# NikoBiele/RayTraceHeatTransfer.jl

Measured on AMD Instinct MI355X. Metric: Mrays/sec (exchange-factor trace), 101×101 grey κ=1 enclosure, 1/2/4/8 GPUs, higher is better.
Workload: dtype f64; 1 GPU; 101x101 grey kappa=1 sigma_s=0 unit-square enclosure (BASELINE configs[1]); 1e+08 rays per GPU, emitter rows sharded over 1 GPU(s); n_emitters=10605, rays_per_emitter=9429, parallelism=emitter-rows x1 (one process per GPU), devices_visible=1, seed=1

## Files before the change

raytraceheattransfer.jl_amd/csrc/rthx_api.cpp:

```cpp
#define RTHX_HOST_ONLY_TU 1
#include <hip/hip_runtime.h>

#include <algorithm>
#include <array>
#include <chrono>
#include <cmath>
#include <cstdio>
#include <cstdlib>
#include <cstring>
#include <map>
#include <mutex>
#include <string>
#include <thread>
#include <vector>

#include "../../include/rthx.h"
#include "rthx_grid.h"
#include "rthx_kernels.h"

#include "rthx_common.h"
#include "rthx_domain.h"

using rthx::DevBuf;
using rthx::HostBuf;
// ... 144 lines not shown
extern "C" __attribute__((visibility("default"))) int rthx_debug_neg_log(const double* u, int64_t n, double* out) {
  if ((!u || !out) && n > 0) return -1;
  std::vector<double> t(rthx::kTableDoubles);
  rthx::fill_tables(t.data());
  for (int64_t k = 0; k < n; ++k) out[k] = rthx::neg_log_tab(u[k], t.data() + rthx::kLogTableOffset);
  return 0;
}

extern "C" __attribute__((visibility("default"))) int rthx_debug_neg_log_u32(const uint32_t* w, int64_t n,
                                                                             double* out) {
  if ((!w || !out) && n > 0) return -1;
  std::vector<double> t(rthx::kTableDoubles);
  rthx::fill_tables(t.data());
  for (int64_t k = 0; k < n; ++k) out[k] = rthx::neg_log_u32(w[k], t.data() + rthx::kLogTableOffset);
  return 0;
}

extern "C" __attribute__((visibility("default"))) int rthx_debug_wall_candidate(double s, double d, int32_t form) {
  const double as = std::fabs(s), ad = std::fabs(d);
  switch (form) {
    case 0: return rthx::wall_candidate(s, d) ? 1 : 0;
    case 1: return (ad >= 1e-10 && as * ad > 0.0) ? 1 : 0;
    case 2: return (as / ad > 0.0 && ad >= 1e-10) ? 1 : 0;
    default: return -1;
  }
}

extern "C" __attribute__((visibility("default"))) int rthx_debug_sin_theta_sweep(int32_t device, uint32_t w_begin,
                                                                                 uint64_t n, uint64_t* n_diff,
                                                                                 uint64_t* first_diff) {
  if (!n_diff || !first_diff) return fail(RTHX_EINVAL, "null output");
  if ((uint64_t)w_begin + n > (1ull << 32)) return fail(RTHX_EINVAL, "word range past 2^32");
  hipStream_t stream = nullptr;
  RTHX_TRY(rthx::open_device(device, &stream));
  DevBuf buf;
  HIP_TRY(buf.reserve(2 * sizeof(unsigned long long)), "hipMalloc (sin theta sweep)");
  unsigned long long h[2] = {0ull, ~0ull};
  HIP_TRY(hipMemcpyAsync(buf.p, h, sizeof(h), hipMemcpyHostToDevice, stream), "hipMemcpy (sin theta sweep)");
  HIP_TRY(rthx::launch_sin_theta_sweep(w_begin, n, (unsigned long long*)buf.p, stream), "sin_theta_sweep_kernel");
  HIP_TRY(hipMemcpyAsync(h, buf.p, sizeof(h), hipMemcpyDeviceToHost, stream), "hipMemcpy (sin theta sweep)");
  HIP_TRY(hipStreamSynchronize(stream), "hipStreamSynchronize (sin theta sweep)");
  *n_diff = h[0];
  *first_diff = h[1];
  return RTHX_OK;
}

// ... 435 lines not shown
      const int w2 = (w + 1) % dom->c_nv[c];
      const std::pair<double, double> a{v[2 * w], v[2 * w + 1]}, b{v[2 * w2], v[2 * w2 + 1]};
      return a < b ? Key{a.first, a.second, b.first, b.second} : Key{b.first, b.second, a.first, a.second};
    };
    std::map<Key, std::vector<std::pair<size_t, int>>> walls;
    for (size_t c = 0; c < nc; ++c)
      for (int w = 0; w < dom->c_nv[c]; ++w) walls[key_of(c, w)].push_back({c, w});
    const std::vector<uint32_t> flagged = mask;
    for (size_t c = 0; c < nc; ++c)
      for (int w = 0; w < dom->c_nv[c]; ++w)
        if ((flagged[c] >> w) & 1u)
          for (const auto& o : walls[key_of(c, w)])
            if (!((dom->c_solid[o.first] >> o.second) & 1u)) mask[o.first] |= 1u << o.second;
  }
  rthx::DeviceGuard keep_device;
  HIP_TRY(hipSetDevice(dom->device), "hipSetDevice");
  HIP_TRY(hipMemcpyAsync(dom->d_mirror, mask.data(), nc * sizeof(uint32_t), hipMemcpyHostToDevice, dom->stream),
          "hipMemcpy mirror masks");
  HIP_TRY(hipStreamSynchronize(dom->stream), "mirror masks");
  dom->n_mirror = n;
  return RTHX_OK;
}

RTHX_EXPORT int rthx_domain_get_mirror_walls(const rthx_domain* dom, int64_t* n_mirror) {
  if (!dom || !n_mirror) return fail(RTHX_EINVAL, "null domain or output");
  *n_mirror = dom->n_mirror;
  return RTHX_OK;
}

RTHX_EXPORT void rthx_domain_destroy(rthx_domain* dom) {
  if (!dom) return;
  (void)hipSetDevice(dom->device);
  (void)hipStreamSynchronize(dom->stream);
  delete dom;
}

RTHX_EXPORT int rthx_result_create(rthx_result** out) {
  if (!out) return fail(RTHX_EINVAL, "null out");
  *out = new (std::nothrow) rthx_result();
  return *out ? RTHX_OK : fail(RTHX_ENOMEM, "host allocation failed");
}

RTHX_EXPORT void rthx_result_destroy(rthx_result* res) { delete res; }

namespace rthx {

// ... 111 lines not shown
             p.cl_offset + (size_t)dom->D.cl.bytes + rthx::kStaticLdsBytes <= rthx::kMaxLdsBytes && !no_clds) {
    p.clds = 1;
    p.lds_bytes = p.cl_offset + (size_t)dom->D.cl.bytes;
  }
  if (single && dom->D.lat.bytes > 0 && !p.recording &&
      p.cl_offset + (size_t)dom->D.lat.bytes + rthx::kStaticLdsBytes <= rthx::kMaxLdsBytes) {
    p.clds = 1;
    p.lds_bytes = p.cl_offset + (size_t)dom->D.lat.bytes;
  }
  if (p.n_rows * p.split >= (1ll << 31)) return fail(RTHX_ERANGE, "too many workgroups in one call");
  p.uniform = dom->uniform_beta[a->bin] > -0.1;
  return RTHX_OK;
}

rthx::LaunchCfg launch_of(const rthx_domain* dom, const rthx_trace_args* a, const TracePlan& p) {
  rthx::LaunchCfg L{};
  L.D = dom->d_dom;
  L.lds_bytes = p.lds_bytes;
  L.uniform = p.uniform;
  L.tally = p.tally;
  L.threads = (int)env_int("RTHX_TRACE_THREADS", 0, 0, rthx::kMaxTraceThreads);
  L.faithful = (a->flags & RTHX_FLAG_FAITHFUL_SAMPLING) != 0;
  L.mirror = p.mirror;
  L.single = dom->single_convex && !p.mirror;
  L.clds = p.clds;
  L.axis = dom->axis_rect && !p.mirror && !env_flag("RTHX_NO_AXIS");
  L.T.split = (int32_t)p.split;
  L.T.n_rows = p.n_rows;
  L.rec.n = p.recording ? 1 : 0;
  return L;
}

int plan_trace_split(const rthx_domain* dom, const rthx_trace_args* a, TracePlan& p) {
  int rc = plan_trace(dom, a, p);
  if (rc || p.split > 1 || p.recording || p.n_rows == 0 || p.R < 2 * kSplitMinRays) return rc;
  int64_t slots = 0;
  rthx::LaunchCfg L = launch_of(dom, a, p);
  L.slots = &slots;
  HIP_TRY(rthx::launch_trace(L), "trace kernel occupancy query");
  if (slots <= 0) return RTHX_OK;
  return plan_trace(dom, a, p, slots);
}

int run_trace(rthx_domain* dom, const rthx_trace_args* a, const TracePlan& p, rthx_result* res, bool lookback,
              const rthx::RecordParams& rec, int64_t totals[rthx::kLbTotals], float* ms_trace, float* ms_pack,
              bool async = false, bool check_prev = false) {
// ... 730 lines not shown
```

raytraceheattransfer.jl_amd/csrc/rthx_device.h:

```cpp
#pragma once

#include <hip/hip_runtime.h>
#include <stdint.h>

#if defined(__HIP_DEVICE_COMPILE__) && !defined(RTHX_HOST_ONLY_TU)
#define RTHX_GLOBAL __attribute__((address_space(1)))
#else
#define RTHX_GLOBAL
#endif
#define RTHX_LDS __attribute__((address_space(3)))

namespace rthx {

struct DevGrid {
  double ox, oy;
  double inv_x, inv_y;
  int32_t nx, ny;
  int32_t cell_base;
  int32_t reserved;
};

struct alignas(16) DevPoly {
  double x[4], y[4];
  double nx[4], ny[4];
// ... 199 lines not shown
constexpr uint64_t kLogOff = 0x3FE6000000000000ull;

__host__ __device__ __forceinline__ double neg_log_tab(double u, const double* tab) {
  const uint64_t ix = dbits(u);
  const uint64_t tmp = ix - kLogOff;
  const int i = (int)((tmp >> 45) & (kLogTable - 1));
  const int32_t k = (int32_t)(uint32_t)(tmp >> 32) >> 20;
  const double z = bitsd(ix - (tmp & 0xFFF0000000000000ull));
  const double invc = tab[4 * i], t_hi = tab[4 * i + 1], t_lo = tab[4 * i + 2];
  const double r = __builtin_fma(z, invc, -1.0);
  double q = __builtin_fma(r, 1.0 / 7.0, -1.0 / 6.0);
  q = __builtin_fma(r, q, sconst(1.0 / 5.0));
  q = __builtin_fma(r, q, -1.0 / 4.0);
  q = __builtin_fma(r, q, sconst(1.0 / 3.0));
  q = __builtin_fma(r, q, -0.5);
  const double l1p = __builtin_fma(r * r, q, r);
  const double kd = (double)k;
  const double hi = __builtin_fma(-kd, 6.93147180369123816490e-01, t_hi);
  const double lo = __builtin_fma(-kd, 1.90821492927058770002e-10, t_lo) - l1p;
  const double v = hi + lo;
  return u > 0.0 ? v : __builtin_inf();
}

__host__ __device__ __forceinline__ double neg_log_u32(uint32_t w, const double* tab) {
  static_assert((uint32_t)kLogOff == 0u, "the high-word form needs a zero low word");
  const uint64_t ix = dbits((double)w);
  const uint32_t ix_hi = (uint32_t)(ix >> 32);
  const uint32_t tmp_hi = ix_hi - (uint32_t)(kLogOff >> 32);
  const uint32_t i32 = ((tmp_hi >> 13) & (uint32_t)(kLogTable - 1)) << 5;
  const int32_t k = ((int32_t)tmp_hi >> 20) - 32;
  const double z = bitsd(((uint64_t)(ix_hi - (tmp_hi & 0xFFF00000u)) << 32) | (uint32_t)ix);
  const double* const te = (const double*)((const char*)tab + i32);
  const double invc = te[0], t_hi = te[1], t_lo = te[2];
  const double r = __builtin_fma(z, invc, -1.0);
  double q = fma_cc(r, 1.0 / 7.0, -1.0 / 6.0);
  q = __builtin_fma(r, q, sconst(1.0 / 5.0));
  q = __builtin_fma(r, q, -1.0 / 4.0);
  q = __builtin_fma(r, q, sconst(1.0 / 3.0));
  q = __builtin_fma(r, q, -0.5);
  const double l1p = __builtin_fma(r * r, q, r);
  const double kd = (double)k;
  const double hi = __builtin_fma(-kd, 6.93147180369123816490e-01, t_hi);
  const double lo = __builtin_fma(-kd, 1.90821492927058770002e-10, t_lo) - l1p;
  const double v = hi + lo;
  return w != 0u ? v : __builtin_inf();
}

__device__ __forceinline__ double div_pos(double n, double d) {
  double r = __builtin_amdgcn_rcp(d);
  double e = __builtin_fma(-d, r, 1.0);
  r = __builtin_fma(r, e, r);
  e = __builtin_fma(-d, r, 1.0);
  r = __builtin_fma(r, e, r);
  const double q = n * r;
  const double rem = __builtin_fma(-d, q, n);
  return __builtin_fma(rem, r, q);
}

__device__ __forceinline__ double sqrt_unit(double x) {
  const double y = __builtin_amdgcn_rsq(__builtin_fmax(x, 0x1.0p-1000));
  double g = x * y, h = 0.5 * y;
  const double r = __builtin_fma(-h, g, 0.5);
  g = __builtin_fma(g, r, g);
  h = __builtin_fma(h, r, h);
  double d = __builtin_fma(-g, g, x);
  g = __builtin_fma(d, h, g);
  d = __builtin_fma(-g, g, x);
// ... 554 lines not shown
  bool gas;
  bool lost;
  bool cold;
};

__device__ __forceinline__ int lattice_walk(const double RTHX_LDS* b, int nm1, int i, double x) {
#pragma unroll 1
  while (true) {
    const bool dn = i > 0 && x < b[i];
    const bool up = !dn && i < nm1 && !(x < b[i + 1]);
    if (!(dn | up)) break;
    i += dn ? -1 : 1;
  }
  return (b[i] <= x && x < b[i + 1]) ? i : -1;
}

__device__ __forceinline__ int lattice_guess(double x, double x0, double inv, int nm1) {
  int i;
  __asm__("v_cvt_i32_f64 %0, %1" : "=v"(i) : "v"(__dmul_rn(x - x0, inv)));
  __asm__("v_med3_i32 %0, %1, 0, %2" : "=v"(i) : "v"(i), "v"(nm1));
  return i;
}

template <bool INSIDE>
__device__ __forceinline__ int lat_ray_fast(const DevDomain& D, double eta, const SingleCoarse& sc,
                                            const char RTHX_LDS* lat_base, bool identity, bool cold0, LatRay& r) {
  const double ox = r.px, oy = r.py, dx = r.dx, dy = r.dy, S = r.S;
  const double cx0 = sc.poly.x[0], cx1 = sc.poly.x[1], cy0 = sc.poly.y[0], cy1 = sc.poly.y[2];
  const bool xdn = dx < 0.0, ydn = dy < 0.0;
  const bool y_first = ydn | xdn;
  double u;
  int k;
  if (INSIDE) {
    const double xb = xdn ? cx0 : cx1, yb = ydn ? cy0 : cy1;
    const double sx = xb - ox, sy = yb - oy;
    const bool vx = wall_candidate(sx, dx), vy = wall_candidate(sy, dy);
    const double cx = __dmul_rn(fabs(sx), fabs(dy)), cy = __dmul_rn(fabs(sy), fabs(dx));
    const bool xw = vx & (!vy | (y_first & (cx < cy)) | (!y_first & !(cy < cx)));
    const bool any = vx | vy;
    const double q = div_pos(fabs(xw ? sx : sy), fabs(xw ? dx : dy));
    u = any ? q : __builtin_inf();
    k = any ? (xw ? (xdn ? 3 : 1) : (ydn ? 0 : 2)) : 0;
  } else {
    if (cx0 <= ox && ox < cx1 && cy0 <= oy && oy < cy1)
      u = dist_in_box(ox, oy, dx, dy, xdn ? cx0 : cx1, ydn ? cy0 : cy1, k);
    else
      u = dist_to_box(ox, oy, dx, dy, cx0, cx1, cy0, cy1, k);
  }
  const bool gas = S < u;
  const bool wall = !gas & (((sc.solid >> k) & 1u) != 0u);
  const bool lost = !(gas | wall);
  const double t = (gas ? S : u) - eta;
  const double px = ox + __dmul_rn(t, dx);
  const double py = oy + __dmul_rn(t, dy);
  r.px = px;
  r.py = py;
  r.gas = gas;
  r.lost = lost;
  const LatGrid& G = sc.lat;
  const double RTHX_LDS* xs = (const double RTHX_LDS*)lat_base;
  const double RTHX_LDS* ys = (const double RTHX_LDS*)(lat_base + G.off_ys);
  const int i = lattice_guess(px, G.x0, G.inv_x, G.nxm1);
  const int j = lattice_guess(py, G.y0, G.inv_y, G.nym1);
  const double xlo = xs[i], xhi = xs[i + 1], ylo = ys[j], yhi = ys[j + 1];
  const bool hit = (xlo <= px) & (px < xhi) & (ylo <= py) & (py < yhi);
  int f = lat_cell(i, j, G.nx);
  if (!identity) f = D.lat_map[f];
  const double sx = (xdn ? xlo : xhi) - px, sy = (ydn ? ylo : yhi) - py;
  const bool vx = wall_candidate(sx, dx), vy = wall_candidate(sy, dy);
  const double cx = __dmul_rn(fabs(sx), fabs(dy)), cy = __dmul_rn(fabs(sy), fabs(dx));
  const bool xw = vx & (!vy | (y_first & (cx < cy)) | (!y_first & !(cy < cx)));
  const int wl = xw ? (xdn ? 3 : 1) : (ydn ? 0 : 2);
  int surf = -1;
  if (wall) surf = ld_off32(D.f_surf, ((uint32_t)f << 4) + ((uint32_t)wl << 2));
  const int a = gas ? sc.n_surfaces + f : surf;
  r.cold = cold0 | lost | !hit | (wall & !(vx | vy)) | (a < 0);
  return a;
}

__device__ __forceinline__ int lat_ray_fixup(const DevDomain& D, const SingleCoarse& sc,
                                             const char RTHX_LDS* lat_base, bool identity, const LatRay& r) {
  if (r.lost) return -1;
  const double px = r.px, py = r.py, dx = r.dx, dy = r.dy;
  const LatGrid& G = sc.lat;
  const double RTHX_LDS* xs = (const double RTHX_LDS*)lat_base;
  const double RTHX_LDS* ys = (const double RTHX_LDS*)(lat_base + G.off_ys);
  const int i = lattice_walk(xs, G.nxm1, lattice_guess(px, G.x0, G.inv_x, G.nxm1), px);
  const int j = lattice_walk(ys, G.nym1, lattice_guess(py, G.y0, G.inv_y, G.nym1), py);
  if (i < 0 || j < 0) return -1;
  int f = lat_cell(i, j, G.nx);
  if (!identity) f = D.lat_map[f];
  if (r.gas) return sc.n_surfaces + f;
  const int w = box_hit_in(px, py, dx, dy, dx < 0.0 ? xs[i] : xs[i + 1], dy < 0.0 ? ys[j] : ys[j + 1]).wall;
  return ld_off32(D.f_surf, ((uint32_t)f << 4) + ((uint32_t)w << 2));
}

template <class T>
__device__ __forceinline__ T ld(const T RTHX_LDS* p) { return *(const T*)p; }
template <class T>
__device__ __forceinline__ T ld(const T RTHX_GLOBAL* p) { return *p; }
// ... 400 lines not shown
  px = px + __dmul_rn(t, r.dx);
  py = py + __dmul_rn(t, r.dy);
}

__device__ __forceinline__ int end_ml(const DevDomain& D, const MLatLds& L, const MLatLayout& G, const MBox& B,
                                      double px, double py, double dx, double dy, bool gas) {
  const MCoarse m = ld(L.cinfo + L.cmap[B.b]);
  int i, j;
  const int fg = ml_fine(L, G, m, px, py, i, j);
  if (fg < 0) return -1;
  if (gas) return D.n_surfaces + fg;
  const int w = box_hit_in(px, py, dx, dy, dx < 0.0 ? L.xs[i] : L.xs[i + 1], dy < 0.0 ? L.ys[j] : L.ys[j + 1]).wall;
  return D.f_surf[4 * fg + w];
}

template <bool UNIFORM, bool FAITHFUL>
__device__ __forceinline__ double free_path(const TraceParams& P, const double* tabs, double u) {
  if (UNIFORM)
    return FAITHFUL ? (P.beta_uniform > 0 ? -log(u) / P.beta_uniform : __builtin_inf())
                    : neg_log_tab(u, tabs + kLogTableOffset) * tabs[kTabInvBeta];
  return FAITHFUL ? -log(u) : neg_log_tab(u, tabs + kLogTableOffset);
}

template <bool UNIFORM, bool FAITHFUL, bool LATRAY = false>
__device__ __forceinline__ double free_path_u32(const TraceParams& P, const double* tabs, uint32_t w,
                                                const SingleCoarse* sc = nullptr) {
  if (FAITHFUL) return free_path<UNIFORM, true>(P, tabs, u32(w));
  const double l = neg_log_u32(w, tabs + kLogTableOffset);
  if (UNIFORM) return l * (LATRAY ? sc->inv_beta : tabs[kTabInvBeta]);
  return l;
}

template <int EK = kEmitAny>
__device__ __forceinline__ bool emitter_surface(const Emitter& e) { return EK == kEmitAny ? e.surface : false; }

template <int EK = kEmitAny>
__device__ __forceinline__ RayWords ray_words(const TraceParams& P, const Emitter& e, uint32_t g, uint32_t r,
                                              bool have_pw, uint32_t pw, bool faithful) {
  RayWords rw;
  philox_words(r, g, 0u, (uint32_t)P.bin, P.key0, P.key1, rw.a);
  rw.pw = 0u;
  rw.sw = 0u;
  if (!emitter_surface<EK>(e)) {
    if (have_pw) {
      rw.pw = pw;
    } else {
      uint32_t b[4];
      philox_words(r >> 2, g, 1u, (uint32_t)P.bin, P.key0, P.key1, b);
      const uint32_t j = r & 3u;
      rw.pw = j == 0 ? b[0] : j == 1 ? b[1] : j == 2 ? b[2] : b[3];
    }
    if (EK == kEmitVolRect ? faithful : (e.need_sel || (faithful && e.nv == 4))) {
      uint32_t c[4];
      philox_words(r, g, 2u, (uint32_t)P.bin, P.key0, P.key1, c);
      rw.sw = c[0];
    }
  }
  return rw;
}

template <bool UNIFORM, bool FAITHFUL, int EK = kEmitAny, bool LATRAY = false>
__device__ __forceinline__ void start_ray_w(const TraceParams& P, const Emitter& e, const double* tabs,
                                            const RayWords& rw, double& px, double& py, double& dx, double& dy,
                                            double& S, const SingleCoarse* sc = nullptr) {
  const bool surface = emitter_surface<EK>(e);
  if (surface)
    emit_surface<FAITHFUL>(e, P.eta, rw, tabs, px, py, dx, dy);
  else
    emit_volume<FAITHFUL, EK>(e, P.eta, rw, tabs, px, py, dx, dy);
  uint32_t w_surf = rw.a[3], w_vol = rw.pw;
  __asm__ volatile("" : "+v"(w_surf), "+v"(w_vol));
  S = free_path_u32<UNIFORM, FAITHFUL, LATRAY>(P, tabs, surface ? w_surf : w_vol, sc);
}

template <bool UNIFORM, bool FAITHFUL>
__device__ __forceinline__ void start_ray(const TraceParams& P, const Emitter& e, const double* tabs, uint32_t g,
                                          uint32_t r, double& px, double& py, double& dx, double& dy, double& S) {
  const RayWords rw = ray_words(P, e, g, r, false, 0u, FAITHFUL);
  start_ray_w<UNIFORM, FAITHFUL>(P, e, tabs, rw, px, py, dx, dy, S);
}

template <bool UNIFORM, bool FAITHFUL, bool SINGLE, bool AXIS, bool LAT = false, int EK = kEmitAny>
__device__ __forceinline__ int trace_one_w(const DevDomain& D, const TraceParams& P, const Emitter& e,
                                           const SingleCoarse& sc, const double* tabs, const RayWords& rw,
                                           double& ox, double& oy, double& px, double& py,
                                           const char RTHX_LDS* lat_base = nullptr) {
  double dx, dy, S, acc = 0.0;
  start_ray_w<UNIFORM, FAITHFUL, EK>(P, e, tabs, rw, px, py, dx, dy, S);
  ox = px;
  oy = py;
  if (LAT)
    return segment_lat<UNIFORM, EK == kEmitVolRect>(D, P, sc, lattice_lds_view(lat_base, D.lat), D.lat, px, py, dx,
                                                     dy, S, acc);
  int c = e.coarse;
  for (int it = 0; it < (SINGLE ? 1 : 10000); ++it) {
// ... 8 lines not shown
```

raytraceheattransfer.jl_amd/csrc/rthx_kernels.h:

```cpp
#pragma once

#include <hip/hip_runtime.h>
#include <stdint.h>

#include "rthx_device.h"

namespace rthx {

constexpr int kTraceThreads = 256;
constexpr int kMaxTraceThreads = 1024;
constexpr size_t kMaxLdsBytes = 160 * 1024;
constexpr int64_t kStaticLdsBytes = 10240;
constexpr size_t kMaxCoarseLdsBytes = 48 * 1024;

struct RecordParams {
  int32_t n;
  const int64_t* ids;
  uint8_t* ok;
  double* orig;
  double* end;
};

enum Tally : int { kTallyU32 = 0, kTallyU16 = 1, kTallyHash = 2 };

struct TallyParams {
  int64_t n_emitters;
  int64_t n_rows;
  int64_t row_cap;
  int32_t split;
  int32_t cl_offset;
  uint32_t* stage_cols;
  uint32_t* stage_cnt;
  uint32_t* row_nnz;
  uint32_t* row_tallied;
  uint32_t* dense;
// ... 13 lines not shown
  unsigned long long* totals_next;
  int64_t R;
  uint64_t lb_wait_ticks;
  uint32_t lb_epoch;
  uint32_t check_prev;
};

constexpr int kLbEpochShift = 46;
constexpr int kLbTotals = 6;
constexpr uint32_t kLbEpochMax = 0xFFFF;
constexpr unsigned long long kLbValMax = (1ull << kLbEpochShift) - 1;

struct LaunchCfg {
  const DevDomain* D;
  TraceParams P;
  TallyParams T;
  RecordParams rec;
  size_t lds_bytes;
  hipStream_t stream;
  int tally;
  int threads;
  int clds;
  bool uniform, faithful, single, axis;
  bool mirror = false;
  int64_t* slots = nullptr;
};

hipError_t launch_trace(const LaunchCfg& L);
hipError_t launch_counts_to_F(const int64_t* row_off, const uint32_t* cnt, int64_t n_rows, double* vals,
                              hipStream_t stream);
hipError_t launch_compact(const TallyParams& T, hipStream_t stream);
hipError_t launch_part_merge(const TallyParams& T, hipStream_t stream);
hipError_t launch_scan(const uint32_t* row_nnz, const uint32_t* row_tallied, int64_t n_rows, int64_t R,
                       int64_t* row_off, int64_t* totals, hipStream_t stream);
hipError_t launch_pack(const uint32_t* stage_cols, const uint32_t* stage_cnt, int64_t row_cap, const int64_t* row_off,
                       int64_t n_rows, uint32_t* cols, uint32_t* cnt, hipStream_t stream);
hipError_t launch_sin_theta_sweep(uint32_t w_begin, uint64_t n, unsigned long long* out, hipStream_t stream);
hipError_t launch_sin_theta(const uint32_t* words, int64_t n, double* out, hipStream_t stream);

}
```

raytraceheattransfer.jl_amd/csrc/rthx_kernels.hip:

```cpp
#include <hip/hip_runtime.h>
#include <stdint.h>

#include <algorithm>
#include <map>
#include <mutex>

#include "rthx_device.h"
#include "rthx_kernels.h"
#include "rthx_partition.h"
#include "rthx_wave.h"

namespace rthx {

#ifndef RTHX_TRACE_WAVES_PER_EU
#define RTHX_TRACE_WAVES_PER_EU 5
#endif
#ifndef RTHX_LAT_WAVES_PER_EU
#define RTHX_LAT_WAVES_PER_EU 8
#endif
#ifndef RTHX_MULTI_WAVES_PER_EU
#define RTHX_MULTI_WAVES_PER_EU 4
#endif
#define RTHX_ML_VIEW mlat_lds_view(lds_opaque(cl_base), D.ml)
#define RTHX_ML_G D.ml
// ... 264 lines not shown
  uint32_t base = 0, total = 0;
  for (int w = 0; w < n_waves; ++w) {
    const uint32_t ws = wave_sum[w];
    base += w < wave ? ws : 0u;
    total += ws;
  }
  uint32_t *oc, *on;
  out(total, oc, on);
  uint32_t pos = base + incl - c;
  for (uint32_t w = w0; w < (oc ? w1 : w0); ++w) {
    uint32_t bits = bm[w];
    while (bits) {
      const uint32_t a = 32u * w + (uint32_t)(__ffs(bits) - 1);
      bits &= bits - 1u;
      oc[pos] = a;
      on[pos] = hash_count(keys, cnts, cap - 1u, shift, a);
      ++pos;
    }
  }
  return total;
}

template <bool UNIFORM, int TALLY, bool FAITHFUL, bool SINGLE, bool REC, bool SPLIT, bool AXIS, int CL, bool RBASE,
          bool MIRROR = false>
__global__ __launch_bounds__(kMaxTraceThreads) RTHX_TRACE_WAVES void trace_exchange_kernel(const DevDomain* __restrict__ Dp,
                                                                     TraceParams P, TallyParams T,
                                                                     RecordParams rec) {
  static_assert(!MIRROR || (!SINGLE && !AXIS && CL == 0 && !REC), "mirror walls: the general multi-polygon walker only");
  extern __shared__ __attribute__((aligned(16))) uint32_t hist[];
  const DevDomain& D = *Dp;
  __shared__ uint32_t wave_sum[kMaxTraceThreads / 64];
  __shared__ uint32_t s_tallied;
  __shared__ uint32_t s_next;
  __shared__ Emitter s_emit;
  __shared__ SingleCoarse s_single;
  const double* const g_tab = (const double*)((const double RTHX_GLOBAL*)D.tables + (size_t)P.bin * kLdsTableDoubles);

  constexpr bool CLDS = CL != 0;
  constexpr bool MLAT = CL == 2 && !SINGLE;
  const int tid = threadIdx.x;
  const uint32_t bid = blockIdx.x;
  const uint32_t parts = SPLIT ? (uint32_t)T.split : 1u;
  const uint32_t trow = SPLIT ? bid / parts : bid;
  const uint32_t tpart = SPLIT ? bid - trow * parts : 0u;
  const int64_t slot = trow;
  const int64_t part = tpart;
  const uint32_t chunk = SPLIT ? (uint32_t)((P.R + parts - 1) / parts) : (uint32_t)P.R;
  constexpr bool kBase = RBASE || !SINGLE;
  const int64_t ray_base = kBase ? P.ray_base : 0;
  const int64_t p_begin = SPLIT ? (int64_t)(tpart * chunk) : 0;
  const int64_t r_begin = kBase ? ray_base + (p_begin < P.R ? p_begin : P.R) : p_begin;
  const int64_t r_end = kBase ? ray_base + (SPLIT ? (p_begin + chunk < P.R ? p_begin + chunk : P.R) : P.R)
                              : (SPLIT ? (r_begin + chunk < P.R ? r_begin + chunk : P.R) : P.R);
  const int64_t g = P.g_begin + slot * P.g_stride;
  constexpr bool PACK16 = TALLY == kTallyU16, HASH = TALLY == kTallyHash;
  constexpr bool LATRAY = SINGLE && CL != 0 && AXIS && UNIFORM && !RBASE;
// ... 23 lines not shown
      LayerRec* lay = (LayerRec*)(cl_base + D.ml.off_lay);
      const char RTHX_GLOBAL* blob = (const char RTHX_GLOBAL*)D.ml_blob;
      const double RTHX_GLOBAL* cys = (const double RTHX_GLOBAL*)(blob + D.ml.off_cys);
      const uint32_t RTHX_GLOBAL* bs = (const uint32_t RTHX_GLOBAL*)(blob + D.ml.off_bsolid);
      for (int i = tid; i < D.ml.ncy + 2; i += nthr) {
        const bool layer = i >= 1 && i <= D.ml.ncy;
        LayerRec r;
        r.y0 = layer ? cys[i - 1] : __builtin_nan("");
        r.y1 = layer ? cys[i] : __builtin_nan("");
        r.beta = layer ? D.ml_bbeta[(size_t)P.bin * D.n_coarse + i - 1] : 0.0;
        r.solid = layer ? bs[i - 1] : 0u;
        r.pad = 0u;
        lay[i] = r;
      }
    }
  } else if (CLDS) {
    uint4* dst = (uint4*)cl_base;
    for (int i = tid; i < D.cl.blob_bytes / 16; i += nthr) dst[i] = D.c_blob[i];
    double RTHX_LDS* cb = (double RTHX_LDS*)(cl_base + D.cl.off_beta);
    for (int i = tid; i < D.n_coarse; i += nthr) cb[i] = D.c_beta[(size_t)P.bin * D.n_coarse + i];
  }
  if (tid == 0) {
    s_tallied = 0u;
    s_next = (uint32_t)r_begin;
    s_emit = load_emitter(D, g);
    if (SINGLE) {
      s_single.poly = D.c_poly[0];
      s_single.grid = D.f_grid[0];
      s_single.solid = D.c_solid[0];
      s_single.count = D.f_offset[1];
      if (CLDS && AXIS) {
        const char RTHX_GLOBAL* blob = (const char RTHX_GLOBAL*)D.lat_blob;
        LatGrid lg;
        lg.x0 = *(const double RTHX_GLOBAL*)blob;
        lg.y0 = *(const double RTHX_GLOBAL*)(blob + D.lat.off_ys);
        lg.inv_x = D.lat.inv_x;
        lg.inv_y = D.lat.inv_y;
        lg.nxm1 = D.lat.nx - 1;
        lg.nym1 = D.lat.ny - 1;
        lg.nx = D.lat.nx;
        lg.off_ys = D.lat.off_ys;
        s_single.lat = lg;
        s_single.n_surfaces = D.n_surfaces;
        s_single.inv_beta = P.inv_beta_uniform;
      }
    }
// ... 21 lines not shown
      size_t k = (size_t)rec_slot * (size_t)P.R + (size_t)(r - (uint32_t)ray_base);
      rec.ok[k] = a >= 0 ? 1 : 0;
      rec.orig[2 * k] = ox; rec.orig[2 * k + 1] = oy;
      rec.end[2 * k] = px; rec.end[2 * k + 1] = py;
    }
  };
  if (SINGLE) {
    auto one_ray = [&](uint32_t r, bool have_pw, uint32_t pw, auto ek) {
      constexpr int EK = decltype(ek)::value;
      double ox, oy, px, py;
      const SingleCoarse RTHX_LDS* sc = lds_opaque(&s_single);
      const double* tab = g_tab;
      const Emitter RTHX_LDS* em = lds_opaque(&s_emit);
      const Emitter& e = *(const Emitter*)em;
      const RayWords rw = ray_words<EK>(P, e, (uint32_t)g, r, have_pw, pw, FAITHFUL);
      int a = trace_one_w<UNIFORM, FAITHFUL, SINGLE, AXIS, CLDS && AXIS, EK>(
          D, P, e, *(const SingleCoarse*)sc, (const double*)tab, rw, ox, oy, px, py, lds_opaque(cl_base));
      tally(a);
      record(r, a, ox, oy, px, py);
    };
    const bool lat_identity = LATRAY && __builtin_amdgcn_readfirstlane(D.lat.identity) != 0;
    auto one_ray_lat = [&](uint32_t r, uint32_t pw, bool cold0, auto ek) {
      constexpr int EK = decltype(ek)::value;
      const SingleCoarse RTHX_LDS* scl = lds_opaque(&s_single);
      const SingleCoarse& sc = *(const SingleCoarse*)scl;
      const double* tab = g_tab;
      const Emitter RTHX_LDS* em = lds_opaque(&s_emit);
      const Emitter& e = *(const Emitter*)em;
      const RayWords rw = ray_words<EK>(P, e, (uint32_t)g, r, true, pw, FAITHFUL);
      LatRay ry;
      start_ray_w<UNIFORM, FAITHFUL, EK, true>(P, e, (const double*)tab, rw, ry.px, ry.py, ry.dx, ry.dy, ry.S, &sc);
      const char RTHX_LDS* lat = lds_opaque(cl_base);
      int a = lat_ray_fast<EK == kEmitVolRect>(D, P.eta, sc, lat, lat_identity, cold0, ry);
      auto fixup = [&]() {
        int a2 = -1;
        if (!cold0) {
          a2 = lat_ray_fixup(D, sc, lat, lat_identity, ry);
          if (a2 < 0) atomicSub(&s_tallied, 1u);
        }
        return a2;
      };
      if constexpr (HASH) {
        if (ry.cold) a = fixup();
        if (a >= 0) hash_tally(hist, hist + T.hash_cap, (uint32_t)T.hash_cap - 1u, (uint32_t)T.hash_shift, (uint32_t)a);
      } else {
        uint32_t word = PACK16 ? (uint32_t)a >> 1 : (uint32_t)a;
        uint32_t val = PACK16 ? 1u << ((uint32_t)(a & 1) << 4) : 1u;
        if (ry.cold) {
          const int a2 = fixup();
          word = a2 < 0 ? 0u : PACK16 ? (uint32_t)a2 >> 1 : (uint32_t)a2;
          val = a2 < 0 ? 0u : PACK16 ? 1u << ((uint32_t)(a2 & 1) << 4) : 1u;
        }
        atomicAdd(&hist[word], val);
      }
    };
    const uint32_t rb = (uint32_t)r_begin;
    const uint32_t re = (uint32_t)r_end > rb ? (uint32_t)r_end : rb;
    const uint32_t q0 = rb >> 2, q1 = (re + 3u) >> 2;
    const uint32_t nt = (uint32_t)__builtin_amdgcn_readfirstlane(nthr);
    const bool volume = __builtin_amdgcn_readfirstlane((int)lds_opaque(&s_emit)->surface) == 0;
    const bool vrect = volume && __builtin_amdgcn_readfirstlane((int)lds_opaque(&s_emit)->rect) != 0;
// ... 18 lines not shown
          }
#pragma unroll
          for (uint32_t k = 0; k < 4u; ++k) {
            const uint32_t pw = k == 0u ? b[0] : k == 1u ? b[1] : k == 2u ? b[2] : b[3];
            const bool o = k == 0u ? out[0] : k == 1u ? out[1] : k == 2u ? out[2] : out[3];
            one_ray_lat(4u * q + k, pw, o, ek);
          }
        } else {
#pragma unroll
        for (uint32_t k = 0; k < 4u; ++k) {
          uint32_t r = 4u * q + k;
          const uint32_t pw = k == 0u ? b[0] : k == 1u ? b[1] : k == 2u ? b[2] : b[3];
          bool in = true;
          if (edge) {
            __asm__ volatile("" : "+v"(r));
            in = r >= rb && r < re;
          }
          if (in) one_ray(r, true, pw, ek);
        }
        }
      }
    }
    };
    if constexpr (!FAITHFUL) {
      if (vrect)
        rounds(EmitKind<kEmitVolRect>{});
      else
        rounds(EmitKind<kEmitAny>{});
    } else {
      (void)vrect;
      rounds(EmitKind<kEmitAny>{});
    }
  } else if constexpr (MLAT) {
    constexpr uint32_t kRefillQ = RTHX_REFILL_Q;
    const uint32_t lane = lane_id();
    const uint64_t lt_mask = lane == 0 ? 0ull : (~0ull >> (64 - lane));
    double RTHX_LDS* q = (double RTHX_LDS*)(cl_base + D.ml.bytes) + (tid >> 6) * (64 * kRaySlotDoubles);
    __shared__ MBox s_box0;
    if (tid == 0) ml_enter(mlat_lds_view(cl_base, D.ml), D.ml, s_emit.coarse, s_box0);
    __syncthreads();
    uint32_t q_head = 0, q_cnt = 0;
    bool exhausted = false;
    const bool layered = D.ml.ncx == 1;
    double px = 0.0, py = 0.0, S = 0.0, acc = 0.0, u_end = 0.0;
    MRay ry{};
    int it = 0;
    MBox box{};
// ... 525 lines not shown
  std::lock_guard<std::mutex> g(g_occ_mu);
  auto it = g_occ.find(k);
  return it == g_occ.end() ? OccVal{0, 0} : it->second;
}
static void occupancy_cache_put(const void* kern, size_t lds, OccVal v) {
  const OccKey k{kern, lds, occ_device()};
  std::lock_guard<std::mutex> g(g_occ_mu);
  g_occ[k] = v;
}
static int device_cus() {
  static std::mutex mu;
  static std::map<int, int> cus;
  const int d = occ_device();
  std::lock_guard<std::mutex> g(mu);
  auto it = cus.find(d);
  if (it != cus.end()) return it->second;
  int n = 0;
  if (hipDeviceGetAttribute(&n, hipDeviceAttributeMultiprocessorCount, d) != hipSuccess) n = 0;
  cus[d] = n;
  return n;
}

template <bool UNIFORM, int TALLY, bool FAITHFUL, bool SINGLE, bool REC, bool SPLIT, bool AXIS, int CL = 0,
          bool RBASE = false, bool MIRROR = false>
static hipError_t launch_trace_t(const LaunchCfg& L) {
  if constexpr (SINGLE && !RBASE)
    if (L.P.ray_base != 0) return launch_trace_t<UNIFORM, TALLY, FAITHFUL, SINGLE, REC, SPLIT, AXIS, CL, true>(L);
  auto kern = trace_exchange_kernel<UNIFORM, TALLY, FAITHFUL, SINGLE, REC, SPLIT, AXIS, CL, RBASE, MIRROR>;
  const int64_t blocks = L.T.n_rows * (SPLIT ? L.T.split : 1);
  auto lds_for = [&](int t) { return L.lds_bytes + (CL == 2 && !SINGLE ? (size_t)t * kRaySlotBytes : 0); };
  size_t lds_max = L.lds_bytes;
  for (int t = kTraceThreads; t <= kMaxTraceThreads; t *= 2)
    if (lds_for(t) + (size_t)kStaticLdsBytes <= kMaxLdsBytes) lds_max = std::max(lds_max, lds_for(t));
  if (L.threads == 256 || L.threads == 512 || L.threads == 1024) lds_max = std::max(lds_max, lds_for(L.threads));
  if (lds_max > 64 * 1024) {
    hipError_t e = hipFuncSetAttribute((const void*)kern, hipFuncAttributeMaxDynamicSharedMemorySize, (int)lds_max);
    if (e != hipSuccess) return e;
  }
  OccVal occ = occupancy_cache_get((const void*)kern, L.lds_bytes);
  int threads = occ.threads;
  if (threads == 0) {
    int best_waves = 0, best_per_cu = 0;
    threads = kTraceThreads;
    bool queried = true;
    for (int t = kTraceThreads; t <= kMaxTraceThreads; t *= 2) {
      if (lds_for(t) + (size_t)kStaticLdsBytes > kMaxLdsBytes) break;
      int per_cu = 0;
      if (hipOccupancyMaxActiveBlocksPerMultiprocessor(&per_cu, (const void*)kern, t, lds_for(t)) != hipSuccess) {
        queried = false;
        break;
      }
// ... 5 lines not shown
      }
    }
    occ = OccVal{threads, best_per_cu};
    if (queried) occupancy_cache_put((const void*)kern, L.lds_bytes, occ);
  }
  if (L.threads == 256 || L.threads == 512 || L.threads == 1024) threads = L.threads;
  const size_t lds = lds_for(threads);
  if (L.slots) {
    int per_cu = occ.per_cu;
    if (threads != occ.threads || per_cu == 0) {
      hipError_t e = hipOccupancyMaxActiveBlocksPerMultiprocessor(&per_cu, (const void*)kern, threads, lds);
      if (e != hipSuccess) return e;
    }
    *L.slots = (int64_t)per_cu * device_cus();
    return hipSuccess;
  }
  hipLaunchKernelGGL(kern, dim3((unsigned)blocks), dim3(threads), lds, L.stream, L.D, L.P, L.T, L.rec);
  return hipGetLastError();
}

template <bool UNIFORM, int TALLY, bool FAITHFUL, bool AXIS, bool SPLIT>
static hipError_t launch_trace_s(const LaunchCfg& L) {
  if constexpr (AXIS) {
    if (L.single && L.clds) return launch_trace_t<UNIFORM, TALLY, FAITHFUL, true, false, SPLIT, AXIS, 1>(L);
    if (!L.single && L.clds == 2) return launch_trace_t<UNIFORM, TALLY, FAITHFUL, false, false, SPLIT, AXIS, 2>(L);
  }
  if (L.single) return launch_trace_t<UNIFORM, TALLY, FAITHFUL, true, false, SPLIT, AXIS>(L);
  if (L.clds) return launch_trace_t<UNIFORM, TALLY, FAITHFUL, false, false, SPLIT, AXIS, 1>(L);
  return launch_trace_t<UNIFORM, TALLY, FAITHFUL, false, false, SPLIT, AXIS>(L);
}

template <bool UNIFORM, int TALLY, bool FAITHFUL, bool AXIS>
static hipError_t launch_trace_a(const LaunchCfg& L) {
  return L.T.split > 1 ? launch_trace_s<UNIFORM, TALLY, FAITHFUL, AXIS, true>(L)
                       : launch_trace_s<UNIFORM, TALLY, FAITHFUL, AXIS, false>(L);
}

template <bool UNIFORM, int TALLY, bool FAITHFUL>
static hipError_t launch_trace_u(const LaunchCfg& L) {
  if (L.mirror)
    return L.T.split > 1 ? launch_trace_t<UNIFORM, TALLY, FAITHFUL, false, false, true, false, 0, false, true>(L)
                         : launch_trace_t<UNIFORM, TALLY, FAITHFUL, false, false, false, false, 0, false, true>(L);
  if (L.rec.n > 0) {
    if constexpr (TALLY == kTallyHash)
      if (L.T.split > 1) return launch_trace_t<UNIFORM, TALLY, FAITHFUL, false, true, true, false>(L);
    return launch_trace_t<UNIFORM, TALLY, FAITHFUL, false, true, false, false>(L);
// ... 107 lines not shown
```

Before: 167,700 Mrays/s.

## Add closed-enclosure kernel variant that defers rare lattice rays to a cold list

Adds a PLAINK kernel specialization for uniform single-convex lattice domains whose coarse walls are all solid and whose lattice map is the identity. It drops the solid-mask, lost-ray and lat_map checks and folds tie and zero-word cases into a cold flag. Cold rays are queued in a shared list and re-traced by the general path after the main rounds, instead of being fixed up inline in divergent lanes. If the list overflows, the whole row's histogram is cleared and every ray is re-traced, which risks a large cost on rows with many cold rays.

```diff
diff --git a/raytraceheattransfer.jl_amd/csrc/rthx_api.cpp b/raytraceheattransfer.jl_amd/csrc/rthx_api.cpp
--- a/raytraceheattransfer.jl_amd/csrc/rthx_api.cpp
+++ b/raytraceheattransfer.jl_amd/csrc/rthx_api.cpp
@@ -190,6 +190,20 @@
     case 0: return rthx::wall_candidate(s, d) ? 1 : 0;
     case 1: return (ad >= 1e-10 && as * ad > 0.0) ? 1 : 0;
     case 2: return (as / ad > 0.0 && ad >= 1e-10) ? 1 : 0;
+    default: return -1;
+  }
+}
+
+extern "C" __attribute__((visibility("default"))) int rthx_debug_x_wall(int32_t vx, int32_t vy, int32_t y_first,
+                                                                        double cx, double cy, int32_t form) {
+  const bool bx = vx != 0, by = vy != 0, yf = y_first != 0;
+  switch (form) {
+    case 0: {
+      bool tie = false;
+      const bool xw = rthx::x_wall_untied(bx, by, cx, cy, tie);
+      return (xw ? 1 : 0) | (tie ? 2 : 0);
+    }
+    case 1: return (bx & (!by | (yf & (cx < cy)) | (!yf & !(cy < cx)))) ? 1 : 0;
     default: return -1;
   }
 }
@@ -671,6 +685,11 @@
   return RTHX_OK;
 }
 
+extern "C" __attribute__((visibility("default"))) int rthx_debug_lat_plain(const rthx_domain* dom) {
+  if (!dom || dom->D.lat.bytes <= 0 || dom->c_solid.empty()) return -1;
+  return rthx::lat_plain(dom->c_solid[0], dom->D.lat.identity) ? 1 : 0;
+}
+
 RTHX_EXPORT int rthx_domain_get_mirror_walls(const rthx_domain* dom, int64_t* n_mirror) {
   if (!dom || !n_mirror) return fail(RTHX_EINVAL, "null domain or output");
   *n_mirror = dom->n_mirror;
@@ -828,6 +847,7 @@
   L.threads = (int)env_int("RTHX_TRACE_THREADS", 0, 0, rthx::kMaxTraceThreads);
   L.faithful = (a->flags & RTHX_FLAG_FAITHFUL_SAMPLING) != 0;
   L.mirror = p.mirror;
+  L.lat_plain = rthx_debug_lat_plain(dom) == 1;
   L.single = dom->single_convex && !p.mirror;
   L.clds = p.clds;
   L.axis = dom->axis_rect && !p.mirror && !env_flag("RTHX_NO_AXIS");
diff --git a/raytraceheattransfer.jl_amd/csrc/rthx_device.h b/raytraceheattransfer.jl_amd/csrc/rthx_device.h
--- a/raytraceheattransfer.jl_amd/csrc/rthx_device.h
+++ b/raytraceheattransfer.jl_amd/csrc/rthx_device.h
@@ -245,6 +245,7 @@
   return u > 0.0 ? v : __builtin_inf();
 }
 
+template <bool RAW = false>
 __host__ __device__ __forceinline__ double neg_log_u32(uint32_t w, const double* tab) {
   static_assert((uint32_t)kLogOff == 0u, "the high-word form needs a zero low word");
   const uint64_t ix = dbits((double)w);
@@ -266,6 +267,7 @@
   const double hi = __builtin_fma(-kd, 6.93147180369123816490e-01, t_hi);
   const double lo = __builtin_fma(-kd, 1.90821492927058770002e-10, t_lo) - l1p;
   const double v = hi + lo;
+  if (RAW) return v;
   return w != 0u ? v : __builtin_inf();
 }
 
@@ -866,25 +868,35 @@
   return i;
 }
 
-template <bool INSIDE>
+__host__ __device__ __forceinline__ bool x_wall_untied(bool vx, bool vy, double cx, double cy, bool& tie) {
+  tie = cx == cy;
+  return vx & (!vy | (cx < cy));
+}
+
+template <bool INSIDE, bool PLAIN = false, bool DEFER = false>
 __device__ __forceinline__ int lat_ray_fast(const DevDomain& D, double eta, const SingleCoarse& sc,
-                                            const char RTHX_LDS* lat_base, bool identity, bool cold0, LatRay& r) {
+                                            const char RTHX_LDS* lat_base, bool identity, bool cold0, LatRay& r,
+                                            bool cold1 = false) {
   const double ox = r.px, oy = r.py, dx = r.dx, dy = r.dy, S = r.S;
   const double cx0 = sc.poly.x[0], cx1 = sc.poly.x[1], cy0 = sc.poly.y[0], cy1 = sc.poly.y[2];
   const bool xdn = dx < 0.0, ydn = dy < 0.0;
   const bool y_first = ydn | xdn;
   double u;
   int k;
+  bool rare = false;
   if (INSIDE) {
     const double xb = xdn ? cx0 : cx1, yb = ydn ? cy0 : cy1;
     const double sx = xb - ox, sy = yb - oy;
     const bool vx = wall_candidate(sx, dx), vy = wall_candidate(sy, dy);
     const double cx = __dmul_rn(fabs(sx), fabs(dy)), cy = __dmul_rn(fabs(sy), fabs(dx));
-    const bool xw = vx & (!vy | (y_first & (cx < cy)) | (!y_first & !(cy < cx)));
+    bool tie = false;
+    const bool xw = DEFER ? x_wall_untied(vx, vy, cx, cy, tie)
+                          : vx & (!vy | (y_first & (cx < cy)) | (!y_first & !(cy < cx)));
     const bool any = vx | vy;
     const double q = div_pos(fabs(xw ? sx : sy), fabs(xw ? dx : dy));
-    u = any ? q : __builtin_inf();
-    k = any ? (xw ? (xdn ? 3 : 1) : (ydn ? 0 : 2)) : 0;
+    u = DEFER ? q : any ? q : __builtin_inf();
+    if (DEFER) rare = !any | tie;
+    k = PLAIN ? 0 : any ? (xw ? (xdn ? 3 : 1) : (ydn ? 0 : 2)) : 0;
   } else {
     if (cx0 <= ox && ox < cx1 && cy0 <= oy && oy < cy1)
       u = dist_in_box(ox, oy, dx, dy, xdn ? cx0 : cx1, ydn ? cy0 : cy1, k);
@@ -892,8 +904,8 @@
       u = dist_to_box(ox, oy, dx, dy, cx0, cx1, cy0, cy1, k);
   }
   const bool gas = S < u;
-  const bool wall = !gas & (((sc.solid >> k) & 1u) != 0u);
-  const bool lost = !(gas | wall);
+  const bool wall = PLAIN ? !gas : !gas & (((sc.solid >> k) & 1u) != 0u);
+  const bool lost = PLAIN ? false : !(gas | wall);
   const double t = (gas ? S : u) - eta;
   const double px = ox + __dmul_rn(t, dx);
   const double py = oy + __dmul_rn(t, dy);
@@ -909,7 +921,7 @@
   const double xlo = xs[i], xhi = xs[i + 1], ylo = ys[j], yhi = ys[j + 1];
   const bool hit = (xlo <= px) & (px < xhi) & (ylo <= py) & (py < yhi);
   int f = lat_cell(i, j, G.nx);
-  if (!identity) f = D.lat_map[f];
+  if (!PLAIN && !identity) f = D.lat_map[f];
   const double sx = (xdn ? xlo : xhi) - px, sy = (ydn ? ylo : yhi) - py;
   const bool vx = wall_candidate(sx, dx), vy = wall_candidate(sy, dy);
   const double cx = __dmul_rn(fabs(sx), fabs(dy)), cy = __dmul_rn(fabs(sy), fabs(dx));
@@ -919,7 +931,12 @@
   if (wall) surf = ld_off32(D.f_surf, ((uint32_t)f << 4) + ((uint32_t)wl << 2));
   const int a = gas ? sc.n_surfaces + f : surf;
   r.cold = cold0 | lost | !hit | (wall & !(vx | vy)) | (a < 0);
+  if (DEFER) r.cold |= cold1 | rare;
   return a;
+}
+
+__host__ __device__ __forceinline__ bool lat_plain(uint32_t solid, int identity) {
+  return (solid & 0xFu) == 0xFu && identity != 0;
 }
 
 __device__ __forceinline__ int lat_ray_fixup(const DevDomain& D, const SingleCoarse& sc,
@@ -1366,11 +1383,11 @@
   return FAITHFUL ? -log(u) : neg_log_tab(u, tabs + kLogTableOffset);
 }
 
-template <bool UNIFORM, bool FAITHFUL, bool LATRAY = false>
+template <bool UNIFORM, bool FAITHFUL, bool LATRAY = false, bool RAW = false>
 __device__ __forceinline__ double free_path_u32(const TraceParams& P, const double* tabs, uint32_t w,
                                                 const SingleCoarse* sc = nullptr) {
   if (FAITHFUL) return free_path<UNIFORM, true>(P, tabs, u32(w));
-  const double l = neg_log_u32(w, tabs + kLogTableOffset);
+  const double l = neg_log_u32<RAW>(w, tabs + kLogTableOffset);
   if (UNIFORM) return l * (LATRAY ? sc->inv_beta : tabs[kTabInvBeta]);
   return l;
 }
@@ -1403,10 +1420,10 @@
   return rw;
 }
 
-template <bool UNIFORM, bool FAITHFUL, int EK = kEmitAny, bool LATRAY = false>
+template <bool UNIFORM, bool FAITHFUL, int EK = kEmitAny, bool LATRAY = false, bool RAW = false>
 __device__ __forceinline__ void start_ray_w(const TraceParams& P, const Emitter& e, const double* tabs,
                                             const RayWords& rw, double& px, double& py, double& dx, double& dy,
-                                            double& S, const SingleCoarse* sc = nullptr) {
+                                            double& S, const SingleCoarse* sc = nullptr, bool* w_zero = nullptr) {
   const bool surface = emitter_surface<EK>(e);
   if (surface)
     emit_surface<FAITHFUL>(e, P.eta, rw, tabs, px, py, dx, dy);
@@ -1414,7 +1431,13 @@
     emit_volume<FAITHFUL, EK>(e, P.eta, rw, tabs, px, py, dx, dy);
   uint32_t w_surf = rw.a[3], w_vol = rw.pw;
   __asm__ volatile("" : "+v"(w_surf), "+v"(w_vol));
-  S = free_path_u32<UNIFORM, FAITHFUL, LATRAY>(P, tabs, surface ? w_surf : w_vol, sc);
+  if constexpr (RAW) {
+    const uint32_t w = surface ? w_surf : w_vol;
+    S = free_path_u32<UNIFORM, FAITHFUL, LATRAY, true>(P, tabs, w, sc);
+    *w_zero = w == 0u;
+  } else {
+    S = free_path_u32<UNIFORM, FAITHFUL, LATRAY>(P, tabs, surface ? w_surf : w_vol, sc);
+  }
 }
 
 template <bool UNIFORM, bool FAITHFUL>
diff --git a/raytraceheattransfer.jl_amd/csrc/rthx_kernels.h b/raytraceheattransfer.jl_amd/csrc/rthx_kernels.h
--- a/raytraceheattransfer.jl_amd/csrc/rthx_kernels.h
+++ b/raytraceheattransfer.jl_amd/csrc/rthx_kernels.h
@@ -11,6 +11,7 @@
 constexpr int kMaxTraceThreads = 1024;
 constexpr size_t kMaxLdsBytes = 160 * 1024;
 constexpr int64_t kStaticLdsBytes = 10240;
+constexpr int kLatColdList = 128;
 constexpr size_t kMaxCoarseLdsBytes = 48 * 1024;
 
 struct RecordParams {
@@ -70,6 +71,7 @@
   int threads;
   int clds;
   bool uniform, faithful, single, axis;
+  bool lat_plain = false;
   bool mirror = false;
   int64_t* slots = nullptr;
 };
diff --git a/raytraceheattransfer.jl_amd/csrc/rthx_kernels.hip b/raytraceheattransfer.jl_amd/csrc/rthx_kernels.hip
--- a/raytraceheattransfer.jl_amd/csrc/rthx_kernels.hip
+++ b/raytraceheattransfer.jl_amd/csrc/rthx_kernels.hip
@@ -310,16 +310,20 @@
 }
 
 template <bool UNIFORM, int TALLY, bool FAITHFUL, bool SINGLE, bool REC, bool SPLIT, bool AXIS, int CL, bool RBASE,
-          bool MIRROR = false>
+          bool MIRROR = false, bool PLAINK = false>
 __global__ __launch_bounds__(kMaxTraceThreads) RTHX_TRACE_WAVES void trace_exchange_kernel(const DevDomain* __restrict__ Dp,
                                                                      TraceParams P, TallyParams T,
                                                                      RecordParams rec) {
+  static_assert(!PLAINK || (SINGLE && CL != 0 && AXIS && UNIFORM && !RBASE && !FAITHFUL && !REC),
+                "the closed-enclosure copy: uniform LAT rows, ray base 0, no faithful sampling");
   static_assert(!MIRROR || (!SINGLE && !AXIS && CL == 0 && !REC), "mirror walls: the general multi-polygon walker only");
   extern __shared__ __attribute__((aligned(16))) uint32_t hist[];
   const DevDomain& D = *Dp;
   __shared__ uint32_t wave_sum[kMaxTraceThreads / 64];
   __shared__ uint32_t s_tallied;
   __shared__ uint32_t s_next;
+  __shared__ uint32_t s_cold_n;
+  __shared__ uint32_t s_cold[kLatColdList];
   __shared__ Emitter s_emit;
   __shared__ SingleCoarse s_single;
   const double* const g_tab = (const double*)((const double RTHX_GLOBAL*)D.tables + (size_t)P.bin * kLdsTableDoubles);
@@ -389,6 +393,7 @@
   }
   if (tid == 0) {
     s_tallied = 0u;
+    if constexpr (PLAINK) s_cold_n = 0u;
     s_next = (uint32_t)r_begin;
     s_emit = load_emitter(D, g);
     if (SINGLE) {
@@ -456,6 +461,7 @@
     const bool lat_identity = LATRAY && __builtin_amdgcn_readfirstlane(D.lat.identity) != 0;
     auto one_ray_lat = [&](uint32_t r, uint32_t pw, bool cold0, auto ek) {
       constexpr int EK = decltype(ek)::value;
+      constexpr bool PLAIN = PLAINK;
       const SingleCoarse RTHX_LDS* scl = lds_opaque(&s_single);
       const SingleCoarse& sc = *(const SingleCoarse*)scl;
       const double* tab = g_tab;
@@ -463,14 +469,24 @@
       const Emitter& e = *(const Emitter*)em;
       const RayWords rw = ray_words<EK>(P, e, (uint32_t)g, r, true, pw, FAITHFUL);
       LatRay ry;
-      start_ray_w<UNIFORM, FAITHFUL, EK, true>(P, e, (const double*)tab, rw, ry.px, ry.py, ry.dx, ry.dy, ry.S, &sc);
+      bool w_zero = false;
+      if constexpr (PLAIN)
+        start_ray_w<UNIFORM, FAITHFUL, EK, true, true>(P, e, (const double*)tab, rw, ry.px, ry.py, ry.dx, ry.dy, ry.S,
+                                                       &sc, &w_zero);
+      else
+        start_ray_w<UNIFORM, FAITHFUL, EK, true>(P, e, (const double*)tab, rw, ry.px, ry.py, ry.dx, ry.dy, ry.S, &sc);
       const char RTHX_LDS* lat = lds_opaque(cl_base);
-      int a = lat_ray_fast<EK == kEmitVolRect>(D, P.eta, sc, lat, lat_identity, cold0, ry);
+      int a = lat_ray_fast<EK == kEmitVolRect, PLAIN, PLAIN>(D, P.eta, sc, lat, lat_identity, cold0, ry, w_zero);
       auto fixup = [&]() {
         int a2 = -1;
         if (!cold0) {
-          a2 = lat_ray_fixup(D, sc, lat, lat_identity, ry);
-          if (a2 < 0) atomicSub(&s_tallied, 1u);
+          if constexpr (PLAIN) {
+            const uint32_t slot_c = atomicAdd(&s_cold_n, 1u);
+            if (slot_c < (uint32_t)kLatColdList) s_cold[slot_c] = r;
+          } else {
+            a2 = lat_ray_fixup(D, sc, lat, lat_identity, ry);
+            if (a2 < 0) atomicSub(&s_tallied, 1u);
+          }
         }
         return a2;
       };
@@ -535,7 +551,34 @@
       }
     }
     };
-    if constexpr (!FAITHFUL) {
+    if constexpr (PLAINK) {
+      if (vrect)
+        rounds(EmitKind<kEmitVolRect>{});
+      else
+        rounds(EmitKind<kEmitAny>{});
+      __syncthreads();
+      const uint32_t n_cold = s_cold_n;
+      const bool all = n_cold > (uint32_t)kLatColdList;
+      if (all) {
+        for (int64_t w = tid; w < n_words; w += nthr) hist[w] = 0u;
+        if (tid == 0) s_tallied = 0u;
+        __syncthreads();
+      }
+      const uint32_t n_again = all ? re - rb : n_cold;
+      for (uint32_t i = (uint32_t)tid; i < n_again; i += (uint32_t)nthr) {
+        const uint32_t r = all ? rb + i : s_cold[i];
+        double ox, oy, px, py;
+        const SingleCoarse RTHX_LDS* sc = lds_opaque(&s_single);
+        const double* tab = g_tab;
+        const Emitter RTHX_LDS* em = lds_opaque(&s_emit);
+        const Emitter& e = *(const Emitter*)em;
+        const RayWords rw = ray_words<kEmitAny>(P, e, (uint32_t)g, r, false, 0u, FAITHFUL);
+        const int a = trace_one_w<UNIFORM, FAITHFUL, SINGLE, AXIS, true, kEmitAny>(
+            D, P, e, *(const SingleCoarse*)sc, (const double*)tab, rw, ox, oy, px, py, lds_opaque(cl_base));
+        tally(a);
+        if (a < 0) atomicSub(&s_tallied, 1u);
+      }
+    } else if constexpr (!FAITHFUL) {
       if (vrect)
         rounds(EmitKind<kEmitVolRect>{});
       else
@@ -1107,11 +1150,11 @@
 }
 
 template <bool UNIFORM, int TALLY, bool FAITHFUL, bool SINGLE, bool REC, bool SPLIT, bool AXIS, int CL = 0,
-          bool RBASE = false, bool MIRROR = false>
+          bool RBASE = false, bool MIRROR = false, bool PLAINK = false>
 static hipError_t launch_trace_t(const LaunchCfg& L) {
   if constexpr (SINGLE && !RBASE)
     if (L.P.ray_base != 0) return launch_trace_t<UNIFORM, TALLY, FAITHFUL, SINGLE, REC, SPLIT, AXIS, CL, true>(L);
-  auto kern = trace_exchange_kernel<UNIFORM, TALLY, FAITHFUL, SINGLE, REC, SPLIT, AXIS, CL, RBASE, MIRROR>;
+  auto kern = trace_exchange_kernel<UNIFORM, TALLY, FAITHFUL, SINGLE, REC, SPLIT, AXIS, CL, RBASE, MIRROR, PLAINK>;
   const int64_t blocks = L.T.n_rows * (SPLIT ? L.T.split : 1);
   auto lds_for = [&](int t) { return L.lds_bytes + (CL == 2 && !SINGLE ? (size_t)t * kRaySlotBytes : 0); };
   size_t lds_max = L.lds_bytes;
@@ -1163,6 +1206,9 @@
 template <bool UNIFORM, int TALLY, bool FAITHFUL, bool AXIS, bool SPLIT>
 static hipError_t launch_trace_s(const LaunchCfg& L) {
   if constexpr (AXIS) {
+    if constexpr (UNIFORM && !FAITHFUL)
+      if (L.single && L.clds && L.lat_plain && L.P.ray_base == 0)
+        return launch_trace_t<UNIFORM, TALLY, FAITHFUL, true, false, SPLIT, AXIS, 1, false, false, true>(L);
     if (L.single && L.clds) return launch_trace_t<UNIFORM, TALLY, FAITHFUL, true, false, SPLIT, AXIS, 1>(L);
     if (!L.single && L.clds == 2) return launch_trace_t<UNIFORM, TALLY, FAITHFUL, false, false, SPLIT, AXIS, 2>(L);
   }
```

After: 173,400 Mrays/s (median of 6 runs). 3.4% higher.
